# HighCWu/ControlLoRA

Measured on AMD Instinct MI355X. Metric: train images/sec SD-1.5+ControlLoRA 512^2 bs4/GPU, higher is better.
Workload: dtype f16; 1 GPU; configs/fill50k.json on SD-1.5 topology (seeded random weights), 512x512, bs=4/GPU, fp16; hot path = hint encoder + UNet fwd/bwd + adapter AdamW; latents/text embeddings synthetic (VAE/CLIP outside the hot path); global_batch=4, parallelism=dp1, hipgraph=True, allreduce_bytes=24188160, rccl_ranks=1, comm=torch, comm_requested=auto

## Files before the change

controllora_amd/capi.py:

```python
from __future__ import annotations

import ctypes as C
import os
from typing import Optional

import torch

_HERE = os.path.dirname(os.path.abspath(__file__))
LIB_PATH = os.environ.get("CLORA_LIB_PATH") or os.path.join(_HERE, "_build", "libclora.so")

ABI_VERSION = 4
OK, ERR_ARG, ERR_LAUNCH, ERR_WORKSPACE = 0, -1, -2, -3
_ERR = {ERR_ARG: "bad argument", ERR_LAUNCH: "kernel launch failed", ERR_WORKSPACE: "workspace too small"}


class CloraError(RuntimeError):
    pass


class ConvDesc(C.Structure):
    _fields_ = [(n, C.c_int) for n in (
        "enabled", "Hin", "Win", "Cin", "Hout", "Wout", "ksize", "mul", "kmul", "off", "lim_h", "lim_w", "shift",
        "need_even", "kchunk")]

# ... 58 lines not shown
    _fields_ = [("W", C.c_void_p), ("out", C.c_void_p), ("out_t", C.c_void_p), ("ldw", C.c_int), ("ldo", C.c_int), ("ldt", C.c_int),
                ("rows", C.c_int), ("K", C.c_int), ("nmem", C.c_int), ("m", LoraFoldMember * LORA_FOLD_MAX_MEMBERS)]


class LoraWgradJob(C.Structure):
    _fields_ = [("A", C.c_void_p), ("lda", C.c_int), ("T", C.c_void_p), ("ldt", C.c_int), ("toff", C.c_int), ("G", C.c_void_p),
                ("gs_n", C.c_int), ("gs_j", C.c_int), ("M", C.c_int), ("N", C.c_int), ("R", C.c_int), ("scale", C.c_float),
                ("a_rows", C.c_int), ("A2", C.c_void_p), ("lda2", C.c_int)]


class ConvPackJob(C.Structure):
    _fields_ = [("w", C.c_void_p), ("fwd", C.c_void_p), ("dgrad", C.c_void_p), ("Co", C.c_int), ("Ci", C.c_int), ("ksize", C.c_int),
                ("Cip", C.c_int), ("Cop", C.c_int), ("pad_", C.c_int)]


class ConvUnpackJob(C.Structure):
    _fields_ = [("stage", C.c_void_p), ("stage_b", C.c_void_p), ("grad_w", C.c_void_p), ("grad_b", C.c_void_p), ("Co", C.c_int),
                ("Ci", C.c_int), ("ksize", C.c_int), ("Cip", C.c_int)]


LORA_MAX_JOBS = 16
LORA_WGRAD_MAX_JOBS = 32
WGRAD_JOBS_PER_LAUNCH = min(LORA_WGRAD_MAX_JOBS, max(1, int(os.environ.get("CLORA_WGRAD_JOBS", "32"))))
CONV_MAX_JOBS = 32
CANNY_MAX_GROUP = 64
_P, _I, _Z, _F = C.c_void_p, C.c_int, C.c_size_t, C.c_float
_PROTOS = {
    "clora_gemm_f16": [_P, _I, _P, _P, _I, _I, _I, _I, C.POINTER(ConvDesc), C.POINTER(Epilogue), _I, _P, _Z, _P],
    "clora_gemm_f16_ex": [_P, _I, _P, _P, _I, _I, _I, _I, C.POINTER(ConvDesc), C.POINTER(Epilogue), _I, _I, _P, _Z, _P],
    "clora_conv_patch_eligible": [_I, C.POINTER(ConvDesc), _I],
    "clora_conv_strip_eligible": [_I, _I, C.POINTER(ConvDesc)],
    "clora_set_option": [C.c_char_p, _I],
    "clora_conv_wgrad_f16": [_P, _I, _P, _I, _P, _P, _I, _I, _I, C.POINTER(ConvDesc), _I, _P],
    "clora_conv_weight_pack_f32": [_P, _I, _I, _I, _I, _I, _P, _P, _P],
    "clora_conv_wgrad_unpack_f32": [_P, _P, _P, _P, _I, _I, _I, _I, _P],
    "clora_conv_weight_pack_multi_f32": [C.POINTER(ConvPackJob), _I, _P],
    "clora_conv_wgrad_unpack_multi_f32": [C.POINTER(ConvUnpackJob), _I, _P],
    "clora_attn_fwd_f16": [_P, _I, _P, _I, _P, _I, _P, _I, _P, _I, _I, _I, _I, _I, _F, _P],
    "clora_attn_max_head_dim": [_I],
    "clora_attn_fwd_causal_f16": [_P, _I, _P, _I, _P, _I, _P, _I, _I, _I, _I, _I, _F, _P],
    "clora_attn_bwd_f16": [_P, _I, _P, _I, _P, _I, _P, _I, _P, _I, _P, _P, _P, _I, _P, _I, _P, _I, _I, _I, _I, _I, _I, _F, _P, _Z, _P],
    "clora_groupnorm_fwd_f16": [_P, _P, _P, _P, _P, _I, _I, _I, _I, _F, _I, _P, _Z, _P],
    "clora_groupnorm_bwd_f16": [_P, _P, _P, _P, _P, _P, _P, _P, _P, _I, _I, _I, _I, _I, _I, _P, _Z, _P],
    "clora_groupnorm_fwd_f16_ex": [_P, _P, _I, C.POINTER(Deferred), _P, _P, _P, _P, _P, _I, _I, _I, _I, _F, _I, _P, _Z, _P],
    "clora_groupnorm_bwd_f16_ex": [_P, _P, C.POINTER(Deferred), _P, _P, _P, _I, _P, _P, _P, _P, _P, _I, _I, _I, _I, _I, _I, _P, _Z, _P],
    "clora_groupnorm_fwd_f16_team": [_P, _P, _I, C.POINTER(Deferred), _P, _P, _P, _P, _P, _I, _I, _I, _I, _F, _I, _P, _Z, _P, _Z, _P],
    "clora_groupnorm_fwd_f16_lo": [_P, _P, _I, C.POINTER(Deferred), _P, _P, _P, _P, _P, _I, _I, _I, _I, _F, _I, _P, _Z, _P, _Z, _P, _P, _P],
    "clora_layernorm_fwd_f16_lo": [_P, _P, _P, _P, _I, _I, _F, _P, _P],
    "clora_groupnorm_bwd_f16_team": [_P, _P, C.POINTER(Deferred), _P, _P, _P, _I, _P, _P, _P, _P, _P, _I, _I, _I, _I, _I, _I, _P, _Z, _P, _Z, _P],
    "clora_layernorm_bwd_f16_ex": [_P, _P, C.POINTER(Deferred), _P, _P, _P, _I, _I, _F, _P],
    "clora_finish_deferred": [C.POINTER(Deferred), _P],
    "clora_gemm_ln_fusable": [_I, _I, _I, _I, _I],
    "clora_gemm_tile_info": [_I, C.POINTER(GemmTile)],
    "clora_gemm_tile_at": [_I, C.POINTER(GemmTile)],
    "clora_gemm_fused_down_tile": [_I, _I, _I, C.POINTER(_I)],
    "clora_layernorm_fwd_f16": [_P, _P, _P, _P, _I, _I, _F, _P],
    "clora_softmax_rows_f16": [_P, _P, _I, _I, _I, _F, _P],
    "clora_layernorm_bwd_f16": [_P, _P, _P, _P, _P, _I, _I, _F, _P],
    "clora_geglu_fwd_f16": [_P, _P, _I, _I, _P],
    "clora_geglu_bwd_f16": [_P, _P, _P, _I, _I, _P],
    "clora_lora_down_f16": [_P, _I, _P, _I, _P, _I, _I, _I, _I, _I, _I, _I, _I, _F, _P],
    "clora_lora_down_multi_f16": [C.POINTER(LoraDownJob), _I, _P],
    "clora_lora_wgrad_multi_f16": [C.POINTER(LoraWgradJob), _I, _P, _Z, _P],
    "clora_lora_pack_f16": [_P, _I, _I, _P],
    "clora_rank_compose_f32": [C.POINTER(RankSite), _I, _P],
    "clora_rank_mix_f32": [C.POINTER(RankSite), _I, _I, _P, _Z, _P],
# ... 54 lines not shown
        for name, argtypes in _PROTOS.items():
            if not hasattr(self.cdll, name) and os.environ.get("CLORA_ABI_ANY", "") == "1":
                continue
            fn = getattr(self.cdll, name)
            fn.argtypes = argtypes
            fn.restype = C.c_int
        self.cdll.clora_build_info.restype = C.c_char_p
        self.cdll.clora_groupnorm_workspace_bytes.restype = C.c_size_t
        self.cdll.clora_groupnorm_team_state_bytes.restype = C.c_size_t
        self.cdll.clora_lora_wgrad_workspace_bytes.restype = C.c_size_t
        self.cdll.clora_rank_gram_ws_bytes.restype = C.c_size_t
        self._options_from_env()
        self._derived = {}

    def derived(self, key, make):
        if key not in self._derived:
            self._derived[key] = make(self)
        return self._derived[key]

    def tiles(self) -> dict:
        def read(L):
            rows, r = {}, GemmTile()
            while L.cdll.clora_gemm_tile_at(len(rows), C.byref(r)) == OK:
                rows[r.tile_cfg], r = r, GemmTile()
            return rows
        return self.derived("tiles", read)

    _ENV_OPTIONS = {"CLORA_TILE_ORDER": ("tile_order", {"m": 0, "n": 1, "auto": 2, "a": 2, "grid": 3, "g": 3}), "CLORA_LN_ROWS": ("ln_rows", None),
                    "CLORA_ATTN_FWD_WAVES": ("attn_fwd_waves", None), "CLORA_ATTN_BWD_WAVES": ("attn_bwd_waves", None),
                    "CLORA_GN_BLOCKS": ("gn_blocks", None), "CLORA_EPI_TWO_PHASE": ("epi_two_phase", None),
                    "CLORA_LORA_DOWN_MODE": ("lora_down_mode", None), "CLORA_GN_UNROLL": ("gn_unroll", None),
                    "CLORA_EPI_HOIST": ("epi_hoist", None), "CLORA_GN_RESIDENT": ("gn_resident", None),
                    "CLORA_DEFER_MAX_ROWS": ("defer_max_rows", None), "CLORA_WGRAD_PATCH": ("wgrad_patch", None), "CLORA_STRIP_BLOCKS": ("strip_blocks", None),
                    "CLORA_GN_TEAM": ("gn_team", None)}

    def _options_from_env(self):
        for var, (name, names) in self._ENV_OPTIONS.items():
            v = os.environ.get(var)
            if v is None or v == "":
                continue
            try:
                val = names[v] if (names and v in names) else int(v)
                self.call("clora_set_option", name.encode(), val)
            except (ValueError, CloraError) as e:
                allowed = f"one of {sorted(names)} or an integer" if names else "an integer in the range include/clora.h documents"
                raise CloraError(f"environment variable {var}={v!r} is not a valid value for the library option "
                                 f"{name!r} (expected {allowed})") from e

    def call(self, name: str, *args) -> None:
        rc = getattr(self.cdll, name)(*args)
        if rc != OK:
            raise CloraError(f"{name} failed: {_ERR.get(rc, rc)}")


_LIB: Optional[Lib] = None


def lib() -> Lib:
    global _LIB
    if _LIB is None:
        _LIB = Lib()
    return _LIB


def ptr(t: Optional[torch.Tensor], dtype=None) -> Optional[int]:
    if t is None:
        return None
# ... 13 lines not shown
```

controllora_amd/csrc/clora_common.h:

```cpp
#pragma once
#include <hip/hip_runtime.h>
#include <stdint.h>

typedef _Float16 half_t;
typedef _Float16 half2v __attribute__((ext_vector_type(2)));
typedef _Float16 half4v __attribute__((ext_vector_type(4)));
typedef _Float16 half8 __attribute__((ext_vector_type(8)));
typedef float floatx4 __attribute__((ext_vector_type(4)));

#define CLORA_WAVE 64

#define CLORA_OK 0
#define CLORA_ERR_ARG (-1)
#define CLORA_ERR_LAUNCH (-2)
#define CLORA_ERR_WORKSPACE (-3)

#ifndef CLORA_ASYNC_PRIMS
#define CLORA_ASYNC_PRIMS
#define CLORA_GLDS16(gptr, lptr)                                                                      \
    __builtin_amdgcn_global_load_lds((const __attribute__((address_space(1))) void*)(gptr),            \
                                     (__attribute__((address_space(3))) void*)(lptr), 16, 0, 0)
#define CLORA_WAIT_VMCNT(n) asm volatile("s_waitcnt vmcnt(%0)" ::"n"(n) : "memory")
#define CLORA_RAW_BARRIER() __builtin_amdgcn_s_barrier()
typedef __fp16 clora_fp16x4 __attribute__((__vector_size__(4 * sizeof(__fp16))));
__device__ __forceinline__ half4v clora_ds_read_tr16(const half_t* lptr) {
    clora_fp16x4 v = __builtin_amdgcn_ds_read_tr16_b64_v4f16((__attribute__((address_space(3))) clora_fp16x4*)(lptr));
    half4v r;
    __builtin_memcpy(&r, &v, 8);
    return r;
}
#define CLORA_DS_READ_TR16(lptr) clora_ds_read_tr16(lptr)
#define CLORA_EXP2(x) __builtin_amdgcn_exp2f(x)
#define CLORA_RCP(x) __builtin_amdgcn_rcpf(x)
#define CLORA_KEEP(x) asm volatile("" : "+v"(x))
#define CLORA_KEEP_PURE(x) asm("" : "+v"(x))
#define CLORA_FMA_F32(acc, a, b) asm("v_fma_f32 %0, %1, %2, %0" : "+v"(acc) : "v"(a), "v"(b))
#define CLORA_CYCLES() ((unsigned long long)__builtin_readcyclecounter())
#define CLORA_WALL_TICKS() ((unsigned long long)wall_clock64())
#define CLORA_MFMA_INPLACE(acc, a, b) asm volatile("v_mfma_f32_16x16x32_f16 %0, %1, %2, %0" : "+v"(acc) : "v"(a), "v"(b))
#define CLORA_MFMA_DRAIN() asm volatile("s_nop 15\n\ts_nop 15" ::: "memory")
#define CLORA_WAIT_LGKMCNT(n) asm volatile("s_waitcnt lgkmcnt(%0)" ::"n"(n) : "memory")
#define CLORA_SETPRIO(n) __builtin_amdgcn_s_setprio(n)
#define CLORA_SCHED_BARRIER() __builtin_amdgcn_sched_barrier(0)
typedef __attribute__((address_space(1))) unsigned long long clora_gu64;
typedef __attribute__((address_space(1))) unsigned clora_gu32;
#define CLORA_LD_AGENT_U64(p) __hip_atomic_load((clora_gu64*)(p), __ATOMIC_RELAXED, __HIP_MEMORY_SCOPE_AGENT)
#define CLORA_ST_AGENT_U64(p, v) __hip_atomic_store((clora_gu64*)(p), (unsigned long long)(v), __ATOMIC_RELAXED, __HIP_MEMORY_SCOPE_AGENT)
#define CLORA_LD_AGENT_U32(p) __hip_atomic_load((clora_gu32*)(p), __ATOMIC_RELAXED, __HIP_MEMORY_SCOPE_AGENT)
#define CLORA_ST_AGENT_U32(p, v) __hip_atomic_store((clora_gu32*)(p), (unsigned)(v), __ATOMIC_RELAXED, __HIP_MEMORY_SCOPE_AGENT)
#define CLORA_SLEEP() __builtin_amdgcn_s_sleep(1)
#endif
#ifndef CLORA_SEQUENTIAL_BLOCKS
#define CLORA_SEQUENTIAL_BLOCKS 0
#endif

__device__ __forceinline__ floatx4 mfma16(half8 a, half8 b, floatx4 c) {
    return __builtin_amdgcn_mfma_f32_16x16x32_f16(a, b, c, 0, 0, 0);
}

__device__ __forceinline__ half8 ld8(const half_t* p) { return *reinterpret_cast<const half8*>(p); }
__device__ __forceinline__ void st8(half_t* p, half8 v) { *reinterpret_cast<half8*>(p) = v; }
__device__ __forceinline__ half4v ld4(const half_t* p) { return *reinterpret_cast<const half4v*>(p); }
__device__ __forceinline__ void st4(half_t* p, half4v v) { *reinterpret_cast<half4v*>(p) = v; }
__device__ __forceinline__ half8 zero8() {
    half8 z = {0, 0, 0, 0, 0, 0, 0, 0};
    return z;
}
__device__ __forceinline__ floatx4 zero4f() {
    floatx4 z = {0.f, 0.f, 0.f, 0.f};
    return z;
}

__device__ __forceinline__ float sigmoid_f(float x) { return CLORA_RCP(1.0f + CLORA_EXP2(-1.4426950408889634f * x)); }
__device__ __forceinline__ float silu_f(float x) { return x * sigmoid_f(x); }
__device__ __forceinline__ float dsilu_f(float x) {
    float s = sigmoid_f(x);
    return s * (1.0f + x * (1.0f - s));
}
__device__ __forceinline__ void gelu_parts(float x, float& cdf, float& pdf) {
    const float ax = fabsf(x) * 0.70710678118654752f;
    const float t = CLORA_RCP(1.0f + 0.3275911f * ax);
    const float ex = CLORA_EXP2(-1.4426950408889634f * ax * ax);
    const float poly = t * (0.254829592f + t * (-0.284496736f + t * (1.421413741f + t * (-1.453152027f + t * 1.061405429f))));
// ... 1 lines not shown
    cdf = 0.5f * (1.0f + (x < 0.f ? -erf_abs : erf_abs));
    pdf = 0.39894228040143268f * ex;
}
__device__ __forceinline__ float gelu_f(float x) {
    float cdf, pdf;
    gelu_parts(x, cdf, pdf);
    return x * cdf;
}
__device__ __forceinline__ float dgelu_f(float x) {
    float cdf, pdf;
    gelu_parts(x, cdf, pdf);
    return cdf + x * pdf;
}

__device__ __forceinline__ float wave_sum(float v) {
    v += __shfl_xor(v, 32);
    v += __shfl_xor(v, 16);
    v += __shfl_xor(v, 8);
    v += __shfl_xor(v, 4);
    v += __shfl_xor(v, 2);
    v += __shfl_xor(v, 1);
    return v;
}
__device__ __forceinline__ float wave_max(float v) {
    v = fmaxf(v, __shfl_xor(v, 32));
    v = fmaxf(v, __shfl_xor(v, 16));
    v = fmaxf(v, __shfl_xor(v, 8));
    v = fmaxf(v, __shfl_xor(v, 4));
    v = fmaxf(v, __shfl_xor(v, 2));
    v = fmaxf(v, __shfl_xor(v, 1));
    return v;
}

enum { CLORA_OPT_TILE_ORDER = 0, CLORA_OPT_LN_ROWS, CLORA_OPT_ATTN_FWD_WAVES, CLORA_OPT_ATTN_BWD_WAVES, CLORA_OPT_GN_BLOCKS, CLORA_OPT_EPI_TWO_PHASE, CLORA_OPT_LORA_DOWN_MODE, CLORA_OPT_GN_UNROLL, CLORA_OPT_EPI_HOIST, CLORA_OPT_GN_RESIDENT, CLORA_OPT_DEFER_MAX_ROWS, CLORA_OPT_WGRAD_PATCH, CLORA_OPT_STRIP_BLOCKS, CLORA_OPT_GN_TEAM, CLORA_OPT_COUNT };
__attribute__((visibility("hidden"))) int clora_option(int id);
static inline int clora_xcd_policy() { return clora_option(CLORA_OPT_TILE_ORDER); }
static inline int clora_ln_rows() { return clora_option(CLORA_OPT_LN_ROWS); }

static inline int clora_check_launch() { return hipGetLastError() == hipSuccess ? CLORA_OK : CLORA_ERR_LAUNCH; }
static inline int clora_cdiv(long a, long b) { return (int)((a + b - 1) / b); }
```

controllora_amd/csrc/clora_gemm.hip:

```cpp
#include <string.h>
#include "clora_common.h"
#include "../../include/clora.h"
#include "clora_epilogue.h"

namespace {

struct GemmArgs {
    const half_t* A;
    const half_t* B;
    half_t* C;
    float* partial;
    int lda, ldc, M, N, K;
    int k_per_split;
    int tiles_n;
    int two_phase;
    int hoist_on;
    int tiles_m, n_major;
    int xg_s, xg_m, xg_n;
    clora_conv_t conv;
    clora_epilogue_t epi;
};

template <int BM, int BN, int WM, int WN>
__global__ __launch_bounds__(256) void gemm_kernel(GemmArgs p) {
// ... 1258 lines not shown
            for (int j = 0; j < 2; ++j) {
                const half_t* q = Xs + (wn * 2 + j) * SUB + ks * 512 + troff;
                const half4v lo = CLORA_DS_READ_TR16(q), hi = CLORA_DS_READ_TR16(q + 64);
                bf[j] = half8{lo[0], lo[1], lo[2], lo[3], hi[0], hi[1], hi[2], hi[3]};
            }
#pragma unroll
            for (int i = 0; i < 2; ++i)
#pragma unroll
                for (int j = 0; j < 2; ++j) acc[i][j] = mfma16(af[i], bf[j], acc[i][j]);
        }
    }
    CLORA_WAIT_VMCNT(0);
#pragma unroll
    for (int i = 0; i < 2; ++i)
#pragma unroll
        for (int j = 0; j < 2; ++j)
#pragma unroll
            for (int r = 0; r < 4; ++r) {
                const int n = n0 + wm * 32 + i * 16 + 4 * g + r;
                const int kk = k0 + wn * 32 + j * 16 + li;
                if (n < p.N && kk < p.K) {
                    if (p.oihw_ci > 0) {
                        const int cin = p.conv.enabled ? p.conv.Cin : p.K;
                        const int tap = kk / cin, ci = kk - tap * cin;
                        const int taps = p.conv.enabled ? p.conv.ksize * p.conv.ksize : 1;
                        if (ci < p.oihw_ci) atomicAdd(p.dW + ((size_t)n * p.oihw_ci + ci) * taps + tap, acc[i][j][r]);
                    } else {
                        atomicAdd(p.dW + (size_t)n * p.K + kk, acc[i][j][r]);
                    }
                } else if (n < p.N && kk == p.K && p.db) atomicAdd(p.db + n, acc[i][j][r]);
            }
}

struct WgradPatchArgs {
    const half_t* dY;
    const half_t* X;
    float* dW;
    float* db;
    int N, K, H, W, nimg, nseg, rows_per_block, row_chunks;
    int Hin, Win;
};

template <int CIN, int NFW, int TW, int STRIDE = 1>
__global__ __launch_bounds__(CIN / 16 * 128) void conv_wgrad_patch_kernel(WgradPatchArgs p) {
    constexpr int WC = CIN / 16, NW = WC * 2, NP = 2 * NFW;
    constexpr int PW = STRIDE == 1 ? TW + 2 : 2 * TW + 1, PPIX = 3 * PW;
    constexpr int P_NI = (PPIX * 2 + 63) / 64;
    constexpr int PLANE = P_NI * 512;
    constexpr int Y_NI = TW * 2 / 64, YPLANE = TW * 16;
    constexpr int BUF = WC * PLANE + NP * YPLANE;
    constexpr int NI = WC * P_NI + NP * Y_NI, NIW = (NI + NW - 1) / NW;
    constexpr int KS = TW / 32;
    static_assert((2 * BUF + 512) * 2 <= 160 * 1024, "LDS per workgroup");
    __shared__ __attribute__((aligned(16))) half_t smem[2 * BUF + 512];
    const int t = threadIdx.x, w = t >> 6, l = t & 63, g = l >> 4, li = l & 15;
    const int cb = w >> 1, wn = w & 1;
    const half_t* zero_page = reinterpret_cast<const half_t*>(g_clora_zero16);

    int bid = blockIdx.x;
    const int rc = bid % p.row_chunks; bid /= p.row_chunks;
    const int seg = bid % p.nseg, img = bid / p.nseg;
    const int x0 = seg * TW, y_beg = rc * p.rows_per_block;
    const int y_end = (y_beg + p.rows_per_block < p.H) ? y_beg + p.rows_per_block : p.H;

    int kind[NIW], soff[NIW], doff[NIW];
#pragma unroll
// ... 386 lines not shown
    if ((M % (c.Hout * c.Wout)) || (long)M * 64 >= (1L << 31) || (N & 3)) return 0;
    if (c.Cin == 8 && N <= 32) return 802;
    if (c.Cin == 8 && N <= 64) return 804;
    if (c.Cin == 32 && N <= 32) return 3202;
    if (c.Cin == 32 && N <= 64) return 3204;
    if (c.Cin == 64 && N <= 32) return 6402;
    return 0;
}

__global__ __launch_bounds__(256) void conv_weight_pack_kernel(const float* w, int Co, int Ci, int taps, int Cip, int Cop,
                                                               half_t* fwd, half_t* dgrad) {
    const int nf = Co * taps * Cip, nd = dgrad ? Cip * taps * Cop : 0;
    for (int i = blockIdx.x * 256 + threadIdx.x; i < nf + nd; i += gridDim.x * 256) {
        if (i < nf) {
            const int ci = i % Cip, tap = (i / Cip) % taps, co = i / (Cip * taps);
            fwd[i] = ci < Ci ? (half_t)w[((size_t)co * Ci + ci) * taps + tap] : (half_t)0.f;
        } else {
            const int q = i - nf;
            const int co = q % Cop, tap = (q / Cop) % taps, ci = q / (Cop * taps);
            dgrad[q] = (ci < Ci && co < Co) ? (half_t)w[((size_t)co * Ci + ci) * taps + tap] : (half_t)0.f;
        }
    }
}

int conv_mode(const GemmArgs& a, int bk) {
    const clora_conv_t& c = a.conv;
    if (!c.enabled) return 0;
    const int kcs = c.kchunk > 0 ? c.kchunk : c.Cin;
    const bool fast = c.ksize == 3 && c.shift == 0 && c.need_even == 0 && (c.kmul == 1 || c.kmul == -1) &&
                      (kcs % bk) == 0 && (a.k_per_split % bk) == 0 && c.lim_h == c.Hin && c.lim_w == c.Win;
    return fast ? 2 : 1;
}

int g_opts[CLORA_OPT_COUNT] = {3, 1, 0, 0, 512, 1, 1, 0, 1, 1, 4, 1, 512, 2};
int tile_order_mode() { return g_opts[CLORA_OPT_TILE_ORDER]; }

double fabric_model_bytes(int tiles_m, int tiles_n, int splits, double a_panel, double b_panel, bool n_major) {
    const int tiles = tiles_m * tiles_n, nwg = tiles * splits;
    const int inner = n_major ? tiles_m : tiles_n;
    const int xq = nwg >> 3, xr = nwg & 7;
    double bytes = 0.0;
    int beg = 0;
    for (int x = 0; x < 8; ++x) {
        const int end = beg + xq + (x < xr ? 1 : 0);
        for (int sp = beg / tiles; sp * tiles < end && sp < splits; ++sp) {
            const int t0 = (beg > sp * tiles ? beg : sp * tiles) - sp * tiles, t1 = (end < (sp + 1) * tiles ? end : (sp + 1) * tiles) - sp * tiles;
            if (t1 <= t0) continue;
            const int outer = (t1 - 1) / inner - t0 / inner + 1;
            const int inn = (t1 - t0 < inner) ? t1 - t0 : inner;
            bytes += n_major ? outer * b_panel + inn * a_panel : outer * a_panel + inn * b_panel;
        }
        beg = end;
    }
    return bytes;
}

void pick_tile_order(GemmArgs& a, int BM, int BN, int splits, bool patch) {
    a.tiles_m = clora_cdiv(a.M, BM);
    a.n_major = 0;
    a.xg_s = a.xg_m = a.xg_n = 0;
    const int mode = tile_order_mode();
    if (mode == 0 || a.tiles_m == 1 || a.tiles_n == 1) return;
    if (mode == 1) { a.n_major = 1; return; }
    const double kper = patch ? (double)a.k_per_split * 576 : (double)a.k_per_split;
    const double a_panel = a.conv.enabled && a.conv.ksize == 3 ? BM * (kper / 9.0) * 2.0 * 1.5 : BM * kper * 2.0;
    const double b_panel = BN * kper * 2.0;
    const double m_cost = fabric_model_bytes(a.tiles_m, a.tiles_n, splits, a_panel, b_panel, false);
// ... 361 lines not shown
    if (!out || index < 0 || index >= kNumTileRows) return CLORA_ERR_ARG;
    *out = kTileRows[index];
    return CLORA_OK;
}

extern "C" int clora_gemm_fused_down_tile(int M, int lora_seg, int tile_cfg, int* out) {
    if (!out || M <= 0 || lora_seg <= 0) return CLORA_ERR_ARG;
    const clora_gemm_tile_t& r = tile_row(tile_cfg);
    if ((r.caps & kD) && lora_seg % r.bn == 0) *out = tile_cfg;
    else if (lora_seg % tile_row(55).bn == 0) *out = M >= 32768 ? 54 : 55;
    else *out = 43;
    return CLORA_OK;
}

extern "C" int clora_finish_deferred(const clora_deferred_t* d, void* stream) {
    if (!d || !d->partial || !d->C || d->splits <= 1 || d->M <= 0 || d->N <= 0 || (d->N & 7) || (d->ldc & 7)) return CLORA_ERR_ARG;
    GemmArgs a = GemmArgs();
    a.partial = const_cast<float*>(d->partial); a.C = (half_t*)d->C; a.ldc = d->ldc; a.M = d->M; a.N = d->N; a.epi = d->epi;
    a.epi.defer = nullptr;
    return finish_or_defer(a, d->splits, nullptr, (hipStream_t)stream);
}

int clora_option(int id) { return (id >= 0 && id < CLORA_OPT_COUNT) ? g_opts[id] : 0; }

extern "C" int clora_set_option(const char* name, int value) {
    if (!name) return CLORA_ERR_ARG;
    struct Opt { const char* name; int id, lo, hi; };
    static const Opt kOpts[] = {{"tile_order", CLORA_OPT_TILE_ORDER, 0, 3}, {"ln_rows", CLORA_OPT_LN_ROWS, 0, 1},
                                {"attn_fwd_waves", CLORA_OPT_ATTN_FWD_WAVES, 0, 16}, {"attn_bwd_waves", CLORA_OPT_ATTN_BWD_WAVES, 0, 8},
                                {"gn_blocks", CLORA_OPT_GN_BLOCKS, 64, 1 << 16}, {"epi_two_phase", CLORA_OPT_EPI_TWO_PHASE, 0, 1},
                                {"lora_down_mode", CLORA_OPT_LORA_DOWN_MODE, 0, 2}, {"gn_unroll", CLORA_OPT_GN_UNROLL, 0, 1},
                                {"epi_hoist", CLORA_OPT_EPI_HOIST, 0, 1}, {"gn_resident", CLORA_OPT_GN_RESIDENT, 0, 1},
                                {"defer_max_rows", CLORA_OPT_DEFER_MAX_ROWS, 0, 16}, {"wgrad_patch", CLORA_OPT_WGRAD_PATCH, 0, 8192}, {"strip_blocks", CLORA_OPT_STRIP_BLOCKS, 64, 16384},
                                {"gn_team", CLORA_OPT_GN_TEAM, 0, 4}};
    for (const Opt& o : kOpts)
        if (!strcmp(name, o.name)) {
            if (value < o.lo || value > o.hi) return CLORA_ERR_ARG;
            if ((o.id == CLORA_OPT_ATTN_FWD_WAVES && value != 0 && value != 4 && value != 6 && value != 8 && value != 16) ||
                (o.id == CLORA_OPT_ATTN_BWD_WAVES && value != 0 && value != 4 && value != 8)) return CLORA_ERR_ARG;
            g_opts[o.id] = value;
            return CLORA_OK;
        }
    return CLORA_ERR_ARG;
}

extern "C" int clora_conv_strip_eligible(int M, int N, const clora_conv_t* conv) {
    return (conv && strip_plan(M, N, *conv)) ? 1 : 0;
}

extern "C" int clora_conv_patch_eligible(int M, const clora_conv_t* conv, int tile_cfg) {
    const clora_gemm_tile_t& r = tile_row(tile_cfg);
    if (!conv || !is_patch_tile(r)) return 0;
    GemmArgs a;
    a.M = M; a.conv = *conv;
    return patch_eligible(a, r) ? 1 : 0;
}

extern "C" int clora_gemm_f16(const clora_half* A, int lda, const clora_half* B, clora_half* C, int ldc, int M, int N,
                              int K, const clora_conv_t* conv, const clora_epilogue_t* epi, int split_k,
                              void* workspace, size_t workspace_bytes, void* stream) {
    return clora_gemm_f16_ex(A, lda, B, C, ldc, M, N, K, conv, epi, split_k, 0, workspace, workspace_bytes, stream);
}

__global__ __launch_bounds__(256) void conv_wgrad_unpack_kernel(float* stage, float* stage_b, float* gw, float* gb, int Co, int Ci,
                                                                int taps, int Cip) {
    const int nw = Co * taps * Cip;
    for (int i = blockIdx.x * 256 + threadIdx.x; i < nw + (gb ? Co : 0); i += gridDim.x * 256) {
// ... 4 lines not shown
            if (ci < Ci) gw[((size_t)co * Ci + ci) * taps + tap] += v;
        } else {
            const int co = i - nw;
            gb[co] += stage_b[co];
            stage_b[co] = 0.f;
        }
    }
}

extern "C" int clora_conv_wgrad_unpack_f32(float* stage, float* stage_b, float* grad_w, float* grad_b, int Co, int Ci, int ksize,
                                           int Cip, void* stream) {
    if (!stage || !grad_w || Co <= 0 || Ci <= 0 || Cip < Ci || (ksize != 1 && ksize != 3) || ((grad_b == nullptr) != (stage_b == nullptr)))
        return CLORA_ERR_ARG;
    const int taps = ksize * ksize;
    const long total = (long)Co * taps * Cip + (grad_b ? Co : 0);
    int blocks = (int)((total + 255) / 256);
    if (blocks > 2048) blocks = 2048;
    hipLaunchKernelGGL(conv_wgrad_unpack_kernel, dim3(blocks), dim3(256), 0, (hipStream_t)stream, stage, stage_b, grad_w, grad_b,
                       Co, Ci, taps, Cip);
    return clora_check_launch();
}

extern "C" int clora_conv_weight_pack_f32(const float* w, int Co, int Ci, int ksize, int Cip, int Cop, clora_half* fwd,
                                          clora_half* dgrad, void* stream) {
    if (!w || !fwd || Co <= 0 || Ci <= 0 || (ksize != 1 && ksize != 3) || Cip < Ci || (Cip & 7) || (dgrad && (Cop < Co || (Cop & 7))))
        return CLORA_ERR_ARG;
    const int taps = ksize * ksize;
    const long total = (long)Co * taps * Cip + (dgrad ? (long)Cip * taps * Cop : 0);
    int blocks = (int)((total + 255) / 256);
    if (blocks > 2048) blocks = 2048;
    hipLaunchKernelGGL(conv_weight_pack_kernel, dim3(blocks), dim3(256), 0, (hipStream_t)stream, w, Co, Ci, taps, Cip, Cop,
                       (half_t*)fwd, (half_t*)dgrad);
    return clora_check_launch();
}

extern "C" int clora_conv_wgrad_f16(const clora_half* dY, int ldy, const clora_half* X, int ldx, float* dW, float* db,
                                    int M, int N, int K, const clora_conv_t* conv, int oihw_ci, void* stream) {
    if (!dY || !X || !dW || M <= 0 || N <= 0 || K <= 0 || (K & 7) || (N & 7) || (ldy & 7) || oihw_ci < 0) return CLORA_ERR_ARG;
    WgradArgs a;
    a.dY = (const half_t*)dY; a.X = (const half_t*)X; a.dW = dW; a.db = db;
    a.ldy = ldy; a.ldx = ldx; a.M = M; a.N = N; a.K = K; a.oihw_ci = oihw_ci;
    if (conv && conv->enabled) {
        a.conv = *conv;
        if ((conv->Cin & 7) || K != conv->ksize * conv->ksize * conv->Cin || conv->kchunk != 0) return CLORA_ERR_ARG;
    } else {
        a.conv = clora_conv_t();
        a.conv.enabled = 0;
        if (ldx & 7) return CLORA_ERR_ARG;
    }
    if (conv && conv->enabled && clora_option(CLORA_OPT_WGRAD_PATCH) && oihw_ci == 0 && ldy == N) {
        const clora_conv_t& c = *conv;
        const bool s1 = c.ksize == 3 && c.mul == 1 && c.kmul == 1 && c.off == -1 && c.shift == 0 && c.need_even == 0 && c.Hout == c.Hin &&
                        c.Wout == c.Win && c.lim_h == c.Hin && c.lim_w == c.Win && c.Hout > 0 && (M % (c.Hout * c.Wout)) == 0 &&
                        (long)M * (c.Cin > N ? c.Cin : N) < (1L << 31);
        const bool s2 = c.ksize == 3 && c.mul == 2 && c.kmul == 1 && c.off == 0 && c.shift == 0 && c.need_even == 0 && c.Hin == 2 * c.Hout &&
                        c.Win == 2 * c.Wout && c.lim_h == c.Hin && c.lim_w == c.Win && c.Hout > 0 && (M % (c.Hout * c.Wout)) == 0 &&
                        (long)M * 4 * (c.Cin > N ? c.Cin : N) < (1L << 31);
        if ((s1 || s2) && (c.Cin == 32 || c.Cin == 64) && N <= 64) {
            WgradPatchArgs q;
            q.dY = (const half_t*)dY; q.X = (const half_t*)X; q.dW = dW; q.db = db; q.N = N; q.K = K; q.H = c.Hout; q.W = c.Wout;
            q.Hin = c.Hin; q.Win = c.Win;
            q.nimg = M / (c.Hout * c.Wout);
            hipStream_t s = (hipStream_t)stream;
            if (s2) {
                if (c.Cin == 32 && N <= 32 && (c.Wout % 64) == 0) return launch_wgrad_patch<32, 1, 64, 2>(q, s);
                if (c.Cin == 32 && N <= 64 && (c.Wout % 64) == 0) return launch_wgrad_patch<32, 2, 64, 2>(q, s);
                if (c.Cin == 64 && N <= 64 && (c.Wout % 64) == 0) return launch_wgrad_patch<64, 2, 64, 2>(q, s);
            } else {
            if (c.Cin == 32 && N <= 32 && (c.Wout % 128) == 0) return launch_wgrad_patch<32, 1, 128>(q, s);
            if (c.Cin == 32 && N <= 64 && (c.Wout % 128) == 0) return launch_wgrad_patch<32, 2, 128>(q, s);
            if (c.Cin == 32 && N <= 64 && (c.Wout % 64) == 0) return launch_wgrad_patch<32, 2, 64>(q, s);
            if (c.Cin == 64 && N <= 64 && (c.Wout % 64) == 0) return launch_wgrad_patch<64, 2, 64>(q, s);
            }
        }
    }
    a.tiles_n = clora_cdiv(N, 64);
    a.tiles_k = clora_cdiv(K + (db ? 8 : 0), 64);
    const int tiles = a.tiles_n * a.tiles_k;
    int chunks = clora_cdiv(2048, tiles);
    int mpb = clora_cdiv(clora_cdiv(M, chunks), 64) * 64;
    if (mpb < 256) mpb = 256;
    a.m_per_block = mpb;
    hipLaunchKernelGGL(conv_wgrad_kernel, dim3(tiles, clora_cdiv(M, mpb)), dim3(256), 0, (hipStream_t)stream, a);
    return clora_check_launch();
}
```

controllora_amd/kernels.py:

```python
from __future__ import annotations

import ctypes as C
import os
from typing import Optional, Tuple

import torch

from . import capi
from .capi import ConvDesc, Epilogue, ptr

f16, f32 = torch.float16, torch.float32


class KernelProfiler:

    def __init__(self, detail=False):
        self.detail = detail
        self.records = []

    def summary(self):
        torch.cuda.synchronize()
        agg = {}
        for name, e0, e1, fl, by in self.records:
            a = agg.setdefault(name, dict(calls=0, ms=0.0, flops=0.0, bytes=0.0))
# ... 268 lines not shown
    return hit[1].view(x.shape)


_TRUNK_NO_OUT = [False]


class TrunkNoOut:

    def __init__(self, cond: bool = True, norm_reads: bool = False):
        self.cond = bool(cond) and not (norm_reads and _TRUNK_NORMS[0])

    def __enter__(self):
        self.prev = _TRUNK_NO_OUT[0]
        _TRUNK_NO_OUT[0] = self.cond or self.prev
        return self

    def __exit__(self, *exc):
        _TRUNK_NO_OUT[0] = self.prev
        return False


def trunk_lo_wanted() -> bool:
    return TRUNK_LO_MODE == "always" or (TRUNK_LO_MODE in ("infer", "norms") and not torch.is_grad_enabled())


def trunk_norms_wanted() -> bool:
    return TRUNK_LO_MODE == "norms" and not torch.is_grad_enabled()


def conv_patch_eligible(M: int, conv: ConvDesc, tile_cfg: int) -> bool:
    return bool(capi.lib().cdll.clora_conv_patch_eligible(M, C.byref(conv), tile_cfg))


TILE_ORDERS = {"m": 0, "n": 1, "auto": 2, "grid": 3}
DEFAULT_TILE_ORDER = "grid"


def set_option(name: str, value: int) -> None:
    capi.lib().call("clora_set_option", name.encode(), int(value))


def set_tile_order(mode: str) -> None:
    set_option("tile_order", TILE_ORDERS[mode])


def conv_wgrad(dY: torch.Tensor, X: torch.Tensor, M: int, N: int, K: int, conv: Optional[ConvDesc],
               ldx: Optional[int] = None, with_bias: bool = False):
    buf = torch.zeros(N * K + (N if with_bias else 0), dtype=f32, device=dY.device)
    dW, db = buf[:N * K].view(N, K), (buf[N * K:] if with_bias else None)
    _call("clora_conv_wgrad_f16", ptr(dY, f16), N, ptr(X, f16), ldx if ldx is not None else K, ptr(dW), ptr(db), M, N, K,
          C.byref(conv) if conv is not None else None, 0, flops=2.0 * M * N * K)
    return (dW, db) if with_bias else dW


def conv_wgrad_into(dY: torch.Tensor, X: torch.Tensor, M: int, N: int, K: int, conv: Optional[ConvDesc],
                    weight_grad: torch.Tensor, bias_grad: Optional[torch.Tensor]):
    assert weight_grad.dtype == f32 and weight_grad.is_contiguous() and weight_grad.shape[0] == N
    _call("clora_conv_wgrad_f16", ptr(dY, f16), N, ptr(X, f16), K, ptr(weight_grad), ptr(bias_grad, f32) if bias_grad is not None else None,
          M, N, K, C.byref(conv) if conv is not None else None, weight_grad.shape[1], flops=2.0 * M * N * K)


def conv_wgrad_staged(dY, X, M, N, K, conv, stage: torch.Tensor, weight_grad: torch.Tensor, bias_grad: Optional[torch.Tensor], Cip: int):
    assert stage.dtype == f32 and stage.numel() == N * K + N and weight_grad.dtype == f32 and weight_grad.is_contiguous()
    sw, sb = stage[:N * K], stage[N * K:]
    _call("clora_conv_wgrad_f16", ptr(dY, f16), N, ptr(X, f16), K, ptr(sw), ptr(sb), M, N, K,
          C.byref(conv) if conv is not None else None, 0, flops=2.0 * M * N * K)
# ... 594 lines not shown
```

include/clora.h:

```cpp
#ifndef CLORA_H
#define CLORA_H
#include <stddef.h>
#include <stdint.h>

#ifdef __cplusplus
extern "C" {
#endif

#define CLORA_OK 0
#define CLORA_ERR_ARG (-1)
#define CLORA_ERR_LAUNCH (-2)
#define CLORA_ERR_WORKSPACE (-3)

typedef uint16_t clora_half;

typedef struct {
    int enabled;
    int Hin, Win, Cin;
    int Hout, Wout;
    int ksize;
    int mul, kmul, off, lim_h, lim_w, shift, need_even;
    int kchunk;
} clora_conv_t;

// ... 56 lines not shown
    int nst, bk, flags;
    int caps;
} clora_gemm_tile_t;
int clora_gemm_tile_info(int tile_cfg, clora_gemm_tile_t* out);
int clora_gemm_tile_at(int index, clora_gemm_tile_t* out);
int clora_gemm_fused_down_tile(int M, int lora_seg, int tile_cfg, int* out);
int clora_finish_deferred(const clora_deferred_t* d, void* stream);

typedef struct {
    const float* D;
    clora_half* out;
    int ldd, R, K, kmajor;
    float scale;
    int pad_;
} clora_lora_pack_job_t;
int clora_lora_pack_f16(const clora_lora_pack_job_t* table, int njobs, int max_k, void* stream);

int clora_gemm_f16(const clora_half* A, int lda, const clora_half* B, clora_half* C, int ldc,
                   int M, int N, int K, const clora_conv_t* conv, const clora_epilogue_t* epi,
                   int split_k, void* workspace, size_t workspace_bytes, void* stream);
int clora_gemm_f16_ex(const clora_half* A, int lda, const clora_half* B, clora_half* C, int ldc,
                      int M, int N, int K, const clora_conv_t* conv, const clora_epilogue_t* epi,
                      int split_k, int tile_cfg, void* workspace, size_t workspace_bytes, void* stream);

int clora_conv_patch_eligible(int M, const clora_conv_t* conv, int tile_cfg);

int clora_conv_strip_eligible(int M, int N, const clora_conv_t* conv);

int clora_set_option(const char* name, int value);

int clora_conv_wgrad_f16(const clora_half* dY, int ldy, const clora_half* X, int ldx, float* dW, float* db,
                         int M, int N, int K, const clora_conv_t* conv, int oihw_ci, void* stream);

int clora_conv_wgrad_unpack_f32(float* stage, float* stage_b, float* grad_w, float* grad_b, int Co, int Ci, int ksize,
                                int Cip, void* stream);

int clora_conv_weight_pack_f32(const float* w, int Co, int Ci, int ksize, int Cip, int Cop, clora_half* fwd,
                               clora_half* dgrad, void* stream);

#define CLORA_CONV_MAX_JOBS 32
typedef struct {
    const float* w;
    clora_half* fwd;
    clora_half* dgrad;
    int Co, Ci, ksize, Cip, Cop, pad_;
} clora_conv_pack_job_t;
int clora_conv_weight_pack_multi_f32(const clora_conv_pack_job_t* jobs, int njobs, void* stream);
typedef struct {
    float* stage;
    float* stage_b;
    float* grad_w;
    float* grad_b;
    int Co, Ci, ksize, Cip;
} clora_conv_unpack_job_t;
int clora_conv_wgrad_unpack_multi_f32(const clora_conv_unpack_job_t* jobs, int njobs, void* stream);

int clora_attn_fwd_f16(const clora_half* q, int ldq, const clora_half* k, int ldk, const clora_half* v, int ldv,
                       clora_half* o, int ldo, float* lse, int B, int H, int Nq, int Nk, int D, float scale,
                       void* stream);
int clora_attn_max_head_dim(int backward);
int clora_attn_fwd_causal_f16(const clora_half* q, int ldq, const clora_half* k, int ldk, const clora_half* v, int ldv,
                              clora_half* o, int ldo, int B, int H, int N, int D, float scale, void* stream);
int clora_attn_bwd_f16(const clora_half* q, int ldq, const clora_half* k, int ldk, const clora_half* v, int ldv,
                       const clora_half* o, int ldo, const clora_half* dO, int lddo, const float* lse,
                       float* delta, clora_half* dq, int lddq, clora_half* dk, int lddk, clora_half* dv, int lddv,
                       int B, int H, int Nq, int Nk, int D, float scale, void* workspace, size_t workspace_bytes,
// ... 159 lines not shown
```

Baseline: 184.2 images/s.

## Add 128x128-tile split-M conv weight-gradient kernel with triple-buffered LDS pipeline

Adds a new conv/linear weight-gradient kernel that computes 128x128 output tiles per 256-thread block. It splits the reduction (M) dimension across blocks sized toward a target block count and combines partials with atomicAdd. Operands stream through a three-stage global-to-LDS async pipeline and are read with transposed LDS loads plus explicit lgkmcnt fences, replacing the 64x64-tile path for eligible shapes. It is on by default through a new option. The aim is better operand reuse and MFMA utilisation for the large wgrad GEMMs, at the cost of more atomic traffic and one block per CU from the launch bounds.

```diff
diff --git a/controllora_amd/capi.py b/controllora_amd/capi.py
--- a/controllora_amd/capi.py
+++ b/controllora_amd/capi.py
@@ -114,6 +114,7 @@
     "clora_conv_strip_eligible": [_I, _I, C.POINTER(ConvDesc)],
     "clora_set_option": [C.c_char_p, _I],
     "clora_conv_wgrad_f16": [_P, _I, _P, _I, _P, _P, _I, _I, _I, C.POINTER(ConvDesc), _I, _P],
+    "clora_conv_wgrad_wide_eligible": [_I, _I, _I, C.POINTER(ConvDesc), _I],
     "clora_conv_weight_pack_f32": [_P, _I, _I, _I, _I, _I, _P, _P, _P],
     "clora_conv_wgrad_unpack_f32": [_P, _P, _P, _P, _I, _I, _I, _I, _P],
     "clora_conv_weight_pack_multi_f32": [C.POINTER(ConvPackJob), _I, _P],
@@ -234,7 +235,7 @@
                     "CLORA_LORA_DOWN_MODE": ("lora_down_mode", None), "CLORA_GN_UNROLL": ("gn_unroll", None),
                     "CLORA_EPI_HOIST": ("epi_hoist", None), "CLORA_GN_RESIDENT": ("gn_resident", None),
                     "CLORA_DEFER_MAX_ROWS": ("defer_max_rows", None), "CLORA_WGRAD_PATCH": ("wgrad_patch", None), "CLORA_STRIP_BLOCKS": ("strip_blocks", None),
-                    "CLORA_GN_TEAM": ("gn_team", None)}
+                    "CLORA_GN_TEAM": ("gn_team", None), "CLORA_WGRAD_WIDE": ("wgrad_wide", None)}
 
     def _options_from_env(self):
         for var, (name, names) in self._ENV_OPTIONS.items():
diff --git a/controllora_amd/csrc/clora_common.h b/controllora_amd/csrc/clora_common.h
--- a/controllora_amd/csrc/clora_common.h
+++ b/controllora_amd/csrc/clora_common.h
@@ -49,6 +49,15 @@
 #define CLORA_LD_AGENT_U32(p) __hip_atomic_load((clora_gu32*)(p), __ATOMIC_RELAXED, __HIP_MEMORY_SCOPE_AGENT)
 #define CLORA_ST_AGENT_U32(p, v) __hip_atomic_store((clora_gu32*)(p), (unsigned)(v), __ATOMIC_RELAXED, __HIP_MEMORY_SCOPE_AGENT)
 #define CLORA_SLEEP() __builtin_amdgcn_s_sleep(1)
+#define CLORA_DS_READ_TR16_RAW(dst, lptr, off)                                                                     \
+    asm volatile("ds_read_b64_tr_b16 %0, %1 offset:%2"                                                              \
+                 : "=v"(dst) : "v"((unsigned)(size_t)(__attribute__((address_space(3))) const void*)(lptr)), "n"(off) : "memory")
+#define CLORA_LGKM_FENCE8(n, r0, r1, r2, r3, r4, r5, r6, r7)                                                        \
+    asm volatile("s_waitcnt lgkmcnt(%8)" : "+v"(r0), "+v"(r1), "+v"(r2), "+v"(r3), "+v"(r4), "+v"(r5), "+v"(r6), "+v"(r7) : "n"(n) : "memory")
+#endif
+#ifndef CLORA_DS_READ_TR16_RAW
+#define CLORA_DS_READ_TR16_RAW(dst, lptr, off) ((dst) = CLORA_DS_READ_TR16((const char*)(lptr) + (off)))
+#define CLORA_LGKM_FENCE8(n, r0, r1, r2, r3, r4, r5, r6, r7) ((void)0)
 #endif
 #ifndef CLORA_SEQUENTIAL_BLOCKS
 #define CLORA_SEQUENTIAL_BLOCKS 0
@@ -116,7 +125,7 @@
     return v;
 }
 
-enum { CLORA_OPT_TILE_ORDER = 0, CLORA_OPT_LN_ROWS, CLORA_OPT_ATTN_FWD_WAVES, CLORA_OPT_ATTN_BWD_WAVES, CLORA_OPT_GN_BLOCKS, CLORA_OPT_EPI_TWO_PHASE, CLORA_OPT_LORA_DOWN_MODE, CLORA_OPT_GN_UNROLL, CLORA_OPT_EPI_HOIST, CLORA_OPT_GN_RESIDENT, CLORA_OPT_DEFER_MAX_ROWS, CLORA_OPT_WGRAD_PATCH, CLORA_OPT_STRIP_BLOCKS, CLORA_OPT_GN_TEAM, CLORA_OPT_COUNT };
+enum { CLORA_OPT_TILE_ORDER = 0, CLORA_OPT_LN_ROWS, CLORA_OPT_ATTN_FWD_WAVES, CLORA_OPT_ATTN_BWD_WAVES, CLORA_OPT_GN_BLOCKS, CLORA_OPT_EPI_TWO_PHASE, CLORA_OPT_LORA_DOWN_MODE, CLORA_OPT_GN_UNROLL, CLORA_OPT_EPI_HOIST, CLORA_OPT_GN_RESIDENT, CLORA_OPT_DEFER_MAX_ROWS, CLORA_OPT_WGRAD_PATCH, CLORA_OPT_STRIP_BLOCKS, CLORA_OPT_GN_TEAM, CLORA_OPT_WGRAD_WIDE, CLORA_OPT_COUNT };
 __attribute__((visibility("hidden"))) int clora_option(int id);
 static inline int clora_xcd_policy() { return clora_option(CLORA_OPT_TILE_ORDER); }
 static inline int clora_ln_rows() { return clora_option(CLORA_OPT_LN_ROWS); }
diff --git a/controllora_amd/csrc/clora_gemm.hip b/controllora_amd/csrc/clora_gemm.hip
--- a/controllora_amd/csrc/clora_gemm.hip
+++ b/controllora_amd/csrc/clora_gemm.hip
@@ -1314,6 +1314,182 @@
             }
 }
 
+__global__ __launch_bounds__(256, 1) void conv_wgrad_wide_kernel(WgradArgs p) {
+    constexpr int BMR = 64, NST = 3, NS = 8;
+    constexpr int HALF = BMR * 64;
+    constexpr int STAGE = 4 * HALF;
+    __shared__ __attribute__((aligned(16))) half_t smem[NST * STAGE];
+    const int t = threadIdx.x;
+    const int tile = blockIdx.x;
+    const int tn = tile % p.tiles_n, tk = tile / p.tiles_n;
+    const int n0 = tn * 128, k0 = tk * 128;
+    const int mbeg = blockIdx.y * p.m_per_block;
+    const int mend = (mbeg + p.m_per_block < p.M) ? mbeg + p.m_per_block : p.M;
+    const int nst = (mend - mbeg + BMR - 1) / BMR;
+    const bool conv = p.conv.enabled != 0;
+    const half_t* zero_page = reinterpret_cast<const half_t*>(g_clora_zero16);
+    const half_t* one_page = reinterpret_cast<const half_t*>(g_clora_one16);
+
+    const int w = t >> 6, l = t & 63, g = l >> 4, li = l & 15;
+    const int lm = w * 16 + (l >> 3);
+    int ncol[NS / 2], kcol[NS / 2], ky[NS / 2], kx[NS / 2], ci[NS / 2];
+    bool n_ok[NS / 2], k_ok[NS / 2], k_one[NS / 2];
+#pragma unroll
+    for (int q = 0; q < NS / 2; ++q) {
+        const int f = ((l >> 4) & 1) | ((q >> 1) << 1);
+        const int col = (q & 1) * 64 + ((((l & 7) >> 1) ^ f) << 4) + (l & 1) * 8;
+        ncol[q] = n0 + col;
+        kcol[q] = k0 + col;
+        n_ok[q] = ncol[q] < p.N;
+        k_ok[q] = kcol[q] < p.K;
+        k_one[q] = p.db != nullptr && kcol[q] == p.K;
+        ky[q] = 0; kx[q] = 0; ci[q] = kcol[q];
+        if (conv && k_ok[q]) {
+            const int tap = kcol[q] / p.conv.Cin;
+            ci[q] = kcol[q] - tap * p.conv.Cin;
+            ky[q] = tap / p.conv.ksize;
+            kx[q] = tap - ky[q] * p.conv.ksize;
+        }
+    }
+    int mrow = mbeg + lm;
+    auto issue_stage = [&](int buf) {
+        half_t* base = smem + buf * STAGE + w * 16 * 64;
+#pragma unroll
+        for (int rg = 0; rg < 2; ++rg) {
+            const int mr = mrow + rg * 8;
+            const bool mok = mr < mend;
+            size_t xrow = 0;
+            int ty0 = 0, tx0 = 0;
+            if (mok) {
+                if (!conv) {
+                    xrow = (size_t)mr * p.ldx;
+                } else {
+                    const int hw = p.conv.Hout * p.conv.Wout;
+                    const int b = mr / hw, rem = mr - b * hw;
+                    const int yo = rem / p.conv.Wout, xo = rem - yo * p.conv.Wout;
+                    xrow = (size_t)b * p.conv.Hin * p.conv.Win;
+                    ty0 = yo * p.conv.mul + p.conv.off;
+                    tx0 = xo * p.conv.mul + p.conv.off;
+                }
+            }
+#pragma unroll
+            for (int h = 0; h < 2; ++h) {
+                const int q = rg * 2 + h;
+                const half_t* src = (mok && n_ok[q]) ? p.dY + (size_t)mr * p.ldy + ncol[q] : zero_page;
+                CLORA_GLDS16(src, base + h * HALF + rg * 8 * 64);
+            }
+#pragma unroll
+            for (int h = 0; h < 2; ++h) {
+                const int q = rg * 2 + h;
+                const half_t* src = zero_page;
+                if (mok && k_one[q]) src = one_page;
+                else if (mok && k_ok[q]) {
+                    if (!conv) {
+                        src = p.X + xrow + kcol[q];
+                    } else {
+                        const int ty = ty0 + ky[q] * p.conv.kmul, tx = tx0 + kx[q] * p.conv.kmul;
+                        bool ok = ty >= 0 && ty < p.conv.lim_h && tx >= 0 && tx < p.conv.lim_w;
+                        if (p.conv.need_even) ok = ok && (((ty | tx) & 1) == 0);
+                        if (ok) src = p.X + (xrow + (size_t)(ty >> p.conv.shift) * p.conv.Win + (tx >> p.conv.shift)) * p.conv.Cin + ci[q];
+                    }
+                }
+                CLORA_GLDS16(src, base + (2 + h) * HALF + rg * 8 * 64);
+            }
+        }
+        mrow += BMR;
+    };
+
+    const int wm = w >> 1, wn = w & 1;
+    const int troff = (g * 8 + (li >> 2)) * 64 + (l & 3) * 4;
+    int xo[4];
+#pragma unroll
+    for (int i = 0; i < 4; ++i) xo[i] = troff + ((i ^ (((li >> 3) & 1) | ((g & 1) << 1))) << 4);
+    floatx4 acc[4][4];
+#pragma unroll
+    for (int i = 0; i < 4; ++i)
+#pragma unroll
+        for (int j = 0; j < 4; ++j) acc[i][j] = zero4f();
+
+#pragma unroll
+    for (int st = 0; st < NST - 1; ++st) issue_stage(st);
+    int rd = 0, wr = NST - 1;
+    for (int it = 0; it < nst; ++it) {
+        CLORA_WAIT_VMCNT((NST - 2) * NS);
+        CLORA_RAW_BARRIER();
+        issue_stage(wr);
+        wr = (wr + 1 == NST) ? 0 : wr + 1;
+        const half_t* Ys = smem + rd * STAGE + wm * HALF;
+        const half_t* Xs = smem + rd * STAGE + (2 + wn) * HALF;
+        rd = (rd + 1 == NST) ? 0 : rd + 1;
+        half4v al[2][4], ah[2][4], bl[2][4], bh[2][4];
+#pragma unroll
+        for (int ks = 0; ks < 2; ++ks) {
+#pragma unroll
+            for (int i = 0; i < 4; ++i) {
+                if (ks == 0) {
+                    CLORA_DS_READ_TR16_RAW(al[ks][i], Ys + xo[i], 0);
+                    CLORA_DS_READ_TR16_RAW(ah[ks][i], Ys + xo[i], 4 * 64 * 2);
+                } else {
+                    CLORA_DS_READ_TR16_RAW(al[ks][i], Ys + xo[i], 32 * 64 * 2);
+                    CLORA_DS_READ_TR16_RAW(ah[ks][i], Ys + xo[i], 36 * 64 * 2);
+                }
+            }
+#pragma unroll
+            for (int j = 0; j < 4; ++j) {
+                if (ks == 0) {
+                    CLORA_DS_READ_TR16_RAW(bl[ks][j], Xs + xo[j], 0);
+                    CLORA_DS_READ_TR16_RAW(bh[ks][j], Xs + xo[j], 4 * 64 * 2);
+                } else {
+                    CLORA_DS_READ_TR16_RAW(bl[ks][j], Xs + xo[j], 32 * 64 * 2);
+                    CLORA_DS_READ_TR16_RAW(bh[ks][j], Xs + xo[j], 36 * 64 * 2);
+                }
+            }
+        }
+#pragma unroll
+        for (int ks = 0; ks < 2; ++ks) {
+            if (ks == 0) {
+                CLORA_LGKM_FENCE8(15, al[0][0], al[0][1], al[0][2], al[0][3], ah[0][0], ah[0][1], ah[0][2], ah[0][3]);
+                CLORA_LGKM_FENCE8(15, bl[0][0], bl[0][1], bl[0][2], bl[0][3], bh[0][0], bh[0][1], bh[0][2], bh[0][3]);
+            } else {
+                CLORA_LGKM_FENCE8(0, al[1][0], al[1][1], al[1][2], al[1][3], ah[1][0], ah[1][1], ah[1][2], ah[1][3]);
+                CLORA_LGKM_FENCE8(0, bl[1][0], bl[1][1], bl[1][2], bl[1][3], bh[1][0], bh[1][1], bh[1][2], bh[1][3]);
+            }
+            half8 af[4], bf[4];
+#pragma unroll
+            for (int i = 0; i < 4; ++i) {
+                af[i] = half8{al[ks][i][0], al[ks][i][1], al[ks][i][2], al[ks][i][3], ah[ks][i][0], ah[ks][i][1], ah[ks][i][2], ah[ks][i][3]};
+                bf[i] = half8{bl[ks][i][0], bl[ks][i][1], bl[ks][i][2], bl[ks][i][3], bh[ks][i][0], bh[ks][i][1], bh[ks][i][2], bh[ks][i][3]};
+            }
+#pragma unroll
+            for (int i = 0; i < 4; ++i)
+#pragma unroll
+                for (int j = 0; j < 4; ++j) CLORA_MFMA_INPLACE(acc[i][j], af[i], bf[j]);
+        }
+    }
+    CLORA_WAIT_VMCNT(0);
+    CLORA_MFMA_DRAIN();
+    const int cin = p.conv.enabled ? p.conv.Cin : p.K;
+    const int taps = p.conv.enabled ? p.conv.ksize * p.conv.ksize : 1;
+#pragma unroll
+    for (int j = 0; j < 4; ++j) {
+        const int kk = k0 + wn * 64 + j * 16 + li;
+        const int tap = kk / cin, ci_o = kk - tap * cin;
+#pragma unroll
+        for (int i = 0; i < 4; ++i)
+#pragma unroll
+            for (int r = 0; r < 4; ++r) {
+                const int n = n0 + wm * 64 + i * 16 + 4 * g + r;
+                if (n < p.N && kk < p.K) {
+                    if (p.oihw_ci > 0) {
+                        if (ci_o < p.oihw_ci) atomicAdd(p.dW + ((size_t)n * p.oihw_ci + ci_o) * taps + tap, acc[i][j][r]);
+                    } else {
+                        atomicAdd(p.dW + (size_t)n * p.K + kk, acc[i][j][r]);
+                    }
+                } else if (n < p.N && kk == p.K && p.db) atomicAdd(p.db + n, acc[i][j][r]);
+            }
+    }
+}
+
 struct WgradPatchArgs {
     const half_t* dY;
     const half_t* X;
@@ -1766,7 +1942,7 @@
     return fast ? 2 : 1;
 }
 
-int g_opts[CLORA_OPT_COUNT] = {3, 1, 0, 0, 512, 1, 1, 0, 1, 1, 4, 1, 512, 2};
+int g_opts[CLORA_OPT_COUNT] = {3, 1, 0, 0, 512, 1, 1, 0, 1, 1, 4, 1, 512, 2, 1};
 int tile_order_mode() { return g_opts[CLORA_OPT_TILE_ORDER]; }
 
 double fabric_model_bytes(int tiles_m, int tiles_n, int splits, double a_panel, double b_panel, bool n_major) {
@@ -2194,7 +2370,7 @@
                                 {"lora_down_mode", CLORA_OPT_LORA_DOWN_MODE, 0, 2}, {"gn_unroll", CLORA_OPT_GN_UNROLL, 0, 1},
                                 {"epi_hoist", CLORA_OPT_EPI_HOIST, 0, 1}, {"gn_resident", CLORA_OPT_GN_RESIDENT, 0, 1},
                                 {"defer_max_rows", CLORA_OPT_DEFER_MAX_ROWS, 0, 16}, {"wgrad_patch", CLORA_OPT_WGRAD_PATCH, 0, 8192}, {"strip_blocks", CLORA_OPT_STRIP_BLOCKS, 64, 16384},
-                                {"gn_team", CLORA_OPT_GN_TEAM, 0, 4}};
+                                {"gn_team", CLORA_OPT_GN_TEAM, 0, 4}, {"wgrad_wide", CLORA_OPT_WGRAD_WIDE, 0, 8192}};
     for (const Opt& o : kOpts)
         if (!strcmp(name, o.name)) {
             if (value < o.lo || value > o.hi) return CLORA_ERR_ARG;
@@ -2265,6 +2441,23 @@
     hipLaunchKernelGGL(conv_weight_pack_kernel, dim3(blocks), dim3(256), 0, (hipStream_t)stream, w, Co, Ci, taps, Cip, Cop,
                        (half_t*)fwd, (half_t*)dgrad);
     return clora_check_launch();
+}
+
+static int wgrad_wide_plan(int M, int N, int K, bool has_bias, int* m_per_block) {
+    if (N < 128 || K < 128) return 0;
+    const int tiles = clora_cdiv(N, 128) * clora_cdiv(K + (has_bias ? 8 : 0), 128);
+    const int target = clora_option(CLORA_OPT_WGRAD_WIDE) >= 64 ? clora_option(CLORA_OPT_WGRAD_WIDE) : 256;
+    const int chunks = target / tiles > 1 ? target / tiles : 1;
+    int mpb = clora_cdiv(clora_cdiv(M, chunks), 64) * 64;
+    if (mpb < 256) mpb = 256;
+    if (m_per_block) *m_per_block = mpb;
+    return clora_cdiv(M, mpb);
+}
+
+extern "C" int clora_conv_wgrad_wide_eligible(int M, int N, int K, const clora_conv_t* conv, int has_bias) {
+    if (M <= 0 || N <= 0 || K <= 0 || (K & 7) || (N & 7)) return 0;
+    if (conv && conv->enabled && ((conv->Cin & 7) || K != conv->ksize * conv->ksize * conv->Cin || conv->kchunk != 0)) return 0;
+    return wgrad_wide_plan(M, N, K, has_bias != 0, nullptr);
 }
 
 extern "C" int clora_conv_wgrad_f16(const clora_half* dY, int ldy, const clora_half* X, int ldx, float* dW, float* db,
@@ -2307,6 +2500,14 @@
             }
         }
     }
+    int wide_mpb = 0;
+    if (clora_option(CLORA_OPT_WGRAD_WIDE) && wgrad_wide_plan(M, N, K, db != nullptr, &wide_mpb)) {
+        a.tiles_n = clora_cdiv(N, 128);
+        a.tiles_k = clora_cdiv(K + (db ? 8 : 0), 128);
+        a.m_per_block = wide_mpb;
+        hipLaunchKernelGGL(conv_wgrad_wide_kernel, dim3(a.tiles_n * a.tiles_k, clora_cdiv(M, wide_mpb)), dim3(256), 0, (hipStream_t)stream, a);
+        return clora_check_launch();
+    }
     a.tiles_n = clora_cdiv(N, 64);
     a.tiles_k = clora_cdiv(K + (db ? 8 : 0), 64);
     const int tiles = a.tiles_n * a.tiles_k;
diff --git a/controllora_amd/kernels.py b/controllora_amd/kernels.py
--- a/controllora_amd/kernels.py
+++ b/controllora_amd/kernels.py
@@ -324,6 +324,10 @@
     return bool(capi.lib().cdll.clora_conv_patch_eligible(M, C.byref(conv), tile_cfg))
 
 
+def conv_wgrad_wide_chunks(M: int, N: int, K: int, conv: Optional[ConvDesc], with_bias: bool) -> int:
+    return int(capi.lib().cdll.clora_conv_wgrad_wide_eligible(M, N, K, C.byref(conv) if conv is not None else None, int(with_bias)))
+
+
 TILE_ORDERS = {"m": 0, "n": 1, "auto": 2, "grid": 3}
 DEFAULT_TILE_ORDER = "grid"
 
diff --git a/include/clora.h b/include/clora.h
--- a/include/clora.h
+++ b/include/clora.h
@@ -112,6 +112,8 @@
 int clora_conv_wgrad_f16(const clora_half* dY, int ldy, const clora_half* X, int ldx, float* dW, float* db,
                          int M, int N, int K, const clora_conv_t* conv, int oihw_ci, void* stream);
 
+int clora_conv_wgrad_wide_eligible(int M, int N, int K, const clora_conv_t* conv, int has_bias);
+
 int clora_conv_wgrad_unpack_f32(float* stage, float* stage_b, float* grad_w, float* grad_b, int Co, int Ci, int ksize,
                                 int Cip, void* stream);
 
```

Result: no change. 184.3 images/s (median of 2 runs) (+0.1%).
